# Princic-1837592/julia-raytracer

Hardware: AMD Instinct MI355X
Metric: Mrays/s + wall-clock render time, cornellbox 1280×720×256spp (higher is better)
Workload: dtype f32; 1 GPU; cornellbox path 1280x720x256spp; scene=cornellbox, sampler=path, width=1280, height=720, spp=256, bounces=8, batch=256, traversal=near, traversal_requested=auto, bvh=middle, parallelism=1 tile groups x 1 sample ranges + RCCL reduce

## Files before the change

### julia-raytracer_amd/csrc/jt_device.h

```cpp
#pragma once

#include <hip/hip_runtime.h>
#include <stdint.h>

#include "jt_records.h"

namespace jtd {

static constexpr float pif = 3.14159265358979323846f;
static constexpr float ray_eps = 0.0001f;
static constexpr float min_roughness = 0.03f * 0.03f;

struct v2 {
    float x, y;
};
struct v3 {
    float x, y, z;
};
struct v4 {
    float x, y, z, w;
};

__device__ __forceinline__ v2 V2(float x, float y) { return v2{x, y}; }
__device__ __forceinline__ v3 V3(float x, float y, float z) { return v3{x, y, z}; }
__device__ __forceinline__ v4 V4(float x, float y, float z, float w) { return v4{x, y, z, w}; }
__device__ __forceinline__ v3 operator+(v3 a, v3 b) { return V3(a.x + b.x, a.y + b.y, a.z + b.z); }
__device__ __forceinline__ v3 operator-(v3 a, v3 b) { return V3(a.x - b.x, a.y - b.y, a.z - b.z); }
__device__ __forceinline__ v3 operator*(v3 a, v3 b) { return V3(a.x * b.x, a.y * b.y, a.z * b.z); }
__device__ __forceinline__ v3 operator*(v3 a, float s) { return V3(a.x * s, a.y * s, a.z * s); }
__device__ __forceinline__ v3 operator/(v3 a, float s) { return V3(a.x / s, a.y / s, a.z / s); }
__device__ __forceinline__ v3 operator-(v3 a) { return V3(-a.x, -a.y, -a.z); }
__device__ __forceinline__ v4 operator+(v4 a, v4 b) { return V4(a.x + b.x, a.y + b.y, a.z + b.z, a.w + b.w); }
__device__ __forceinline__ v4 operator*(v4 a, float s) { return V4(a.x * s, a.y * s, a.z * s, a.w * s); }
__device__ __forceinline__ bool is_zero(v3 a) { return a.x == 0 && a.y == 0 && a.z == 0; }
__device__ __forceinline__ bool all_finite(v3 a) {
    return __builtin_isfinite(a.x) && __builtin_isfinite(a.y) && __builtin_isfinite(a.z);
}
__device__ __forceinline__ v3 xyz(float4 a) { return V3(a.x, a.y, a.z); }
__device__ __forceinline__ v3 xyz(v4 a) { return V3(a.x, a.y, a.z); }

__device__ __forceinline__ float dot(v3 a, v3 b) { return (a.x * b.x + a.y * b.y) + a.z * b.z; }
__device__ __forceinline__ v3 cross(v3 a, v3 b) {
    return V3(a.y * b.z - a.z * b.y, a.z * b.x - a.x * b.z, a.x * b.y - a.y * b.x);
}
#ifndef JT_SQRT_FORM
#define JT_SQRT_FORM 1
#endif
constexpr unsigned JL_SQRT_LO = 0x10000000u;
constexpr unsigned JL_SQRT_HI = 0x7f800000u;
template <int FORM>
__device__ __forceinline__ float sqrt_fast(float x) {
    if constexpr (FORM == 1) {
        const float y = __builtin_amdgcn_rsqf(x);
        const float s = x * y, h = 0.5f * y;
        return __builtin_fmaf(__builtin_fmaf(-s, s, x), h, s);
    } else if constexpr (FORM == 2) {
        const float s = __builtin_amdgcn_sqrtf(x), h = 0.5f * __builtin_amdgcn_rsqf(x);
        return __builtin_fmaf(__builtin_fmaf(-s, s, x), h, s);
    } else if constexpr (FORM == 3) {
        const float s = __builtin_amdgcn_sqrtf(x);
        const float dn = __uint_as_float(__float_as_uint(s) - 1u), up = __uint_as_float(__float_as_uint(s) + 1u);
        const float rd = __builtin_fmaf(-dn, s, x), ru = __builtin_fmaf(-up, s, x);
        const float t = rd <= 0.0f ? dn : s;
        return ru > 0.0f ? up : t;
    } else {
        const float y = __builtin_amdgcn_rsqf(x);
        float g = x * y, h = 0.5f * y;
        const float e = __builtin_fmaf(-h, g, 0.5f);
        h = __builtin_fmaf(h, e, h);
        g = __builtin_fmaf(g, e, g);
        return __builtin_fmaf(__builtin_fmaf(-g, g, x), h, g);
    }
}
__device__ __forceinline__ float jl_sqrt(float x) {
#if JT_SQRT_FORM
    if (__builtin_expect(__float_as_uint(x) - JL_SQRT_LO < JL_SQRT_HI - JL_SQRT_LO, 1)) return sqrt_fast<JT_SQRT_FORM>(x);
#endif
    return __builtin_sqrtf(x);
}
__device__ __forceinline__ v3 normalize(v3 a) {
    float l = jl_sqrt(dot(a, a));
    return l != 0 ? a / l : a;
}
// ... 400 lines not shown
```

### julia-raytracer_amd/csrc/jt_host.cpp

```cpp
#include <algorithm>
#include <cstdlib>
#include <cstring>
#include <mutex>
#include <string>
#include <thread>
#include <vector>

#include "jt_internal.h"

namespace jt {

static thread_local std::string g_last_error;

void set_error(const std::string& msg) { g_last_error = msg; }
int fail(int status, const std::string& msg) {
    set_error(msg);
    return status;
}

static std::mutex g_opt_mu;
static std::map<std::string, std::string> g_opts;
static const char* const kOptionNames[] = {
    "env_alias",  "features",    "lds_scene",   "lds_stack",  "light_inline", "streams",
    "wait_lanes", "light_lanes", "multi_split", "tile_share",  "test_lds_ring",
};
std::map<std::string, std::string> options_snapshot() {
    std::lock_guard<std::mutex> g(g_opt_mu);
    return g_opts;
}

frame3 inverse_frame(const frame3& f, bool non_rigid) {
    f3 c1 = f.x, c2 = f.y, c3 = f.z;
    f3 m1, m2, m3;
    if (non_rigid) {
        f3 k1 = cross(c2, c3), k2 = cross(c3, c1), k3 = cross(c1, c2);
        f3 a1 = mk3(k1.x, k2.x, k3.x), a2 = mk3(k1.y, k2.y, k3.y), a3 = mk3(k1.z, k2.z, k3.z);
        float det = dot(c1, cross(c2, c3));
        float s = 1.0f / det;
        m1 = a1 * s;
        m2 = a2 * s;
        m3 = a3 * s;
    } else {
        m1 = mk3(c1.x, c2.x, c3.x);
        m2 = mk3(c1.y, c2.y, c3.y);
        m3 = mk3(c1.z, c2.z, c3.z);
    }
    f3 t = (m1 * f.o.x + m2 * f.o.y) + m3 * f.o.z;
    return frame3{m1, m2, m3, -t};
}

struct bbox {
    f3 mn, mx;
};
static inline bbox empty_bbox() {
    const float inf = INFINITY;
    return bbox{mk3(inf, inf, inf), mk3(-inf, -inf, -inf)};
}
static inline bbox merge(const bbox& b, f3 p) {
    return bbox{mk3(jl_min(b.mn.x, p.x), jl_min(b.mn.y, p.y), jl_min(b.mn.z, p.z)),
                mk3(jl_max(b.mx.x, p.x), jl_max(b.mx.y, p.y), jl_max(b.mx.z, p.z))};
}
static inline bbox merge(const bbox& a, const bbox& b) {
    return bbox{mk3(jl_min(a.mn.x, b.mn.x), jl_min(a.mn.y, b.mn.y), jl_min(a.mn.z, b.mn.z)),
                mk3(jl_max(a.mx.x, b.mx.x), jl_max(a.mx.y, b.mx.y), jl_max(a.mx.z, b.mx.z))};
}
static inline f3 center(const bbox& b) { return (b.mn + b.mx) / 2.0f; }
static inline float bbox_area(const bbox& b) {
    f3 s = b.mx - b.mn;
    return ((0.000000000001f + 2 * s.x * s.y) + 2 * s.x * s.z) + 2 * s.y * s.z;
}

struct Builder {
    const std::vector<bbox>& boxes;
    bool hq;
    std::vector<int32_t> prims;
    std::vector<f3> centers;
    std::vector<jt_bvh_node> nodes;
// ... 410 lines not shown
```

### julia-raytracer_amd/csrc/jt_integrator.h

```cpp
#pragma once

#include <hip/hip_runtime.h>

#include "jt_bsdf.h"
#include "jt_device.h"
#include "jt_launch.h"
#include "jt_scene_eval.h"
#include "jt_traverse.h"

#ifndef JT_FUSED_BSDF
#define JT_FUSED_BSDF 1
#endif

namespace jtk {
using namespace jtd;

template <int F>
__device__ __forceinline__ v3 sample_lights(const DScene& S, v3 position, float rl, float rel, v2 ruv) {
    const int light_id = sample_uniform(S.nlights, rl);
    const DLight l = S.lights[light_id - 1];
    const float* cdf = S.cdf + l.cdf_offset;
    if (l.instance >= 0) {
        const int element = l.nguide ? sample_discrete_guided(cdf, l.ncdf, rel, S.guide_t + l.guide_offset,
                                                              S.guide_a + l.guide_offset, l.nguide, l.guide_scale)
// ... 110 lines not shown
    Volume vol;
};

__device__ __forceinline__ bool next_bounce(const DParams& P, Path& st) {
    if (st.bounce() >= P.bounces) return true;
    st.ctl += 1u;
    st.phase = PH_SCENE;
    return false;
}
__device__ __forceinline__ bool next_bounce_retry(const DParams& P, Path& st) {
    if (st.bounce() - 1 >= P.bounces) return true;
    st.phase = PH_SCENE;
    return false;
}
template <int F>
__device__ __forceinline__ bool after_weight(const DParams& P, Path& st) {
    if (is_zero(st.weight<F>()) || !all_finite(st.weight<F>())) return true;
    if (st.bounce() > 3) {
        float rr_prob = jl_min(0.99f, max3(st.weight<F>()));
        if (rand1f(st.rng) >= rr_prob) return true;
        st.set_weight<F>(st.weight<F>() * jl_rcp_weight(rr_prob));
    }
    return next_bounce(P, st);
}
template <int F>
__device__ __forceinline__ bool light_advance(const DScene& S, const DParams& P, Path& st) {
    for (;;) {
        st.li += 1;
        if (st.li >= S.nlights) {
            st.o = st.lq<F>();
            const float pdf = st.pdf * S.light_pick_pdf;
            st.set_weight<F>(st.weight<F>() / (0.5f * st.pb<F>() + 0.5f * pdf));
            return after_weight<F>(P, st);
        }
        const DLight l = S.lights[st.li];
        if (!(F & FT_NOIL) && l.instance >= 0) {
            st.lpdf = 0.0f;
            st.ctl &= (1u << CTL_LC) - 1u;
            st.o = st.lq<F>();
            st.phase = PH_LIGHT;
            return false;
        }
        if ((F & FT_ENV) && l.environment >= 0) st.pdf += env_light_pdf(S, l, st.d);
    }
}
template <int F>
__device__ __forceinline__ bool begin_light_pdf(const DScene& S, const DParams& P, Path& st) {
    st.pdf = 0.0f;
    st.li = -1;
    st.set_lq<F>(st.o);
    return light_advance<F>(S, P, st);
}
template <int F>
__device__ __forceinline__ bool light_hit_add(const DScene& S, Path& st, const Hit& h) {
    const int4 lh = row16<F>(S.light_hit + st.li);
    const DInstShade& is = S.inst_shade[lh.x];
    const fr3 f = frame_from(is.f0, is.f1, is.f2);
    const float4* r = S.light_elems + 5 * (lh.y + h.elem);
    const float4 r0 = r[0], r1 = r[1], r2 = r[2], r3 = r[3];
    const v3 p1 = V3(r0.x, r0.y, r0.z), p2 = V3(r0.w, r1.x, r1.y), p3 = V3(r1.z, r1.w, r2.x);
    const v2 uv = V2(h.u, h.v);
    v3 lposition;
    if (!(F & FT_QUAD) || __float_as_int(r3.z) == KIND_TRI) {
        lposition = transform_point(f, interp_tri(p1, p2, p3, uv));
    } else {
        const float4 r4 = r[4];
        lposition = transform_point(f, interp_quad(p1, p2, p3, V3(r4.x, r4.y, r4.z), uv));
    }
    const v3 en = V3(r2.y, r2.z, r2.w);
    v3 lnormal = __float_as_int(r3.y) ? en : transform_normal(f, en);
    const float area = r3.x;
    v3 dd = lposition - st.lq<F>();
    st.lpdf += dot(dd, dd) / (__builtin_fabsf(dot(lnormal, st.d)) * area);
    st.o = lposition + st.d * 0.001f;
    st.ctl += 1u << CTL_LC;
    return st.lcount() < 100;
}
template <int F>
__device__ __forceinline__ bool light_chain_end(const DScene& S, const DParams& P, Path& st) {
    st.pdf += st.lpdf;
    return light_advance<F>(S, P, st);
}
template <int F>
__device__ __forceinline__ bool light_hit(const DScene& S, const DParams& P, Path& st, const Hit& h) {
    if (h.hit && light_hit_add<F>(S, st, h)) return false;
    return light_chain_end<F>(S, P, st);
}

#ifndef JT_LIGHT_LEAF_STEP
#define JT_LIGHT_LEAF_STEP 1
#endif
#ifndef JT_CHAIN_TAIL
#define JT_CHAIN_TAIL 2
#endif
__host__ __device__ constexpr bool ft_mesh_kernel(int F) { return mesh_family(F); }
template <bool WIDE, int F>
__host__ __device__ constexpr bool chain_tail() {
    return JT_CHAIN_TAIL && !WIDE && !(F & FT_NOIL) && F != FT_NONE && !ft_mesh_kernel(F);
}
template <bool WIDE, bool OVF, bool NCACHE, int F>
__host__ __device__ constexpr bool chain_leaf_step() {
    return JT_LIGHT_LEAF_STEP && !WIDE && !OVF && !NCACHE && !ft_mesh_kernel(F);
}
template <bool WIDE, bool OVF, bool NCACHE, int F>
__host__ __device__ constexpr bool chain_dinv_once() {
    return JT_CHAIN_TAIL >= 2 && chain_tail<WIDE, F>() && chain_leaf_step<WIDE, OVF, NCACHE, F>();
}
// ... 133 lines not shown
        } else {
            float rnl = rand1f(st.rng);
            incoming = sample_delta<F>(sh.mat, sh.normal, outgoing, rnl);
            v3 f = eval_delta<F>(sh.mat, sh.normal, outgoing, incoming);
            float pd = sample_delta_pdf<F>(sh.mat, sh.normal, outgoing, incoming);
            st.set_weight<F>((st.weight<F>() * f) / pd);
        }
        const int mtype = sh.mat.type;
        if ((F & FT_VOL) && (mtype == M_REFRACTIVE || mtype == M_VOLUMETRIC || mtype == M_SUBSURFACE) &&
            dot(sh.normal, outgoing) * dot(sh.normal, incoming) < 0) {
            if (!st.flag(F_VOLUME)) {
                st.set_flag(F_VOLUME);
                st.vol.density = sh.mat.density;
                st.vol.scattering = sh.mat.scattering;
                st.vol.scanisotropy = sh.mat.scanisotropy;
            } else {
                st.clear_flag(F_VOLUME);
            }
        }
        st.o = sh.position;
        st.d = incoming;
        return delta ? after_weight<F>(P, st) : begin_light_pdf<F>(S, P, st);
    }
    v3 outgoing = -st.d;
    v3 position = st.o + st.d * isec.t;
    v3 incoming;
    if (rand1f(st.rng) < 0.5f) {
        (void)rand1f(st.rng);
        v2 rn = rand2f(st.rng);
        incoming = sample_scattering(st.vol, outgoing, rn);
    } else {
        float rl = rand1f(st.rng), rel = rand1f(st.rng);
        v2 ruv = rand2f(st.rng);
        incoming = sample_lights<F>(S, position, rl, rel, ruv);
    }
    if (is_zero(incoming)) return true;
    st.set_weight<F>(st.weight<F>() * eval_scattering(st.vol, outgoing, incoming));
    st.set_pb<F>(sample_scattering_pdf(st.vol, outgoing, incoming));
    st.o = position;
    st.d = incoming;
    return begin_light_pdf<F>(S, P, st);
}

template <int F, class AovT>
__device__ __forceinline__ bool naive_hit(const DScene& S, const DParams& P, Path& st, Hit isec, const AovT& aov,
                                          unsigned& shades) {
    if (!isec.hit) {
        if (st.bounce() > 0 || !P.envhidden)
            st.set_radiance<F>(st.radiance<F>() + st.weight<F>() * eval_environment<F>(S, st.d));
        return true;
    }
    v3 outgoing = -st.d;
    Shading sh;
    eval_shading<F>(S, isec.inst, isec.elem, V2(isec.u, isec.v), outgoing, sh);
    shades++;
    if ((F & FT_OPAC) && sh.mat.opacity < 1 && rand1f(st.rng) >= sh.mat.opacity) {
        if (st.opbounce() > 128) return true;
        st.ctl += 1u << CTL_OPB;
        st.o = sh.position + st.d * 0.01f;
        return next_bounce_retry(P, st);
    }
    if (st.bounce() == 0) {
        st.set_flag(F_HIT);
        aov_update<F>(aov, sh.mat.color, sh.normal);
    }
    st.set_radiance<F>(st.radiance<F>() + st.weight<F>() * (dot(sh.normal, outgoing) >= 0 ? sh.mat.emission : V3(0, 0, 0)));
    v3 incoming, f;
    float p;
    if (sh.mat.roughness != 0) {
        float rnl = rand1f(st.rng);
        v2 rn = rand2f(st.rng);
        incoming = sample_bsdfcos<F>(sh.mat, sh.normal, outgoing, rnl, rn);
        if (is_zero(incoming)) return true;
#if JT_FUSED_BSDF
        eval_bsdfcos_pdf<F>(sh.mat, sh.normal, outgoing, incoming, f, p);
#else
        f = eval_bsdfcos<F>(sh.mat, sh.normal, outgoing, incoming);
        p = sample_bsdfcos_pdf<F>(sh.mat, sh.normal, outgoing, incoming);
#endif
    } else {
        float rnl = rand1f(st.rng);
        incoming = sample_delta<F>(sh.mat, sh.normal, outgoing, rnl);
        if (is_zero(incoming)) return true;
        f = eval_delta<F>(sh.mat, sh.normal, outgoing, incoming);
        p = sample_delta_pdf<F>(sh.mat, sh.normal, outgoing, incoming);
    }
    st.set_weight<F>((st.weight<F>() * f) / p);
    st.o = sh.position;
    st.d = incoming;
    return after_weight<F>(P, st);
}

__device__ __forceinline__ void eval_camera(const DCamera& cam, v2 image_uv, v2 lens_uv, v3& ro, v3& rd) {
    const fr3 frame = frame_from(cam.frame);
    const v2 film = V2(cam.film_x, cam.film_y);
    if (!cam.orthographic) {
        v3 q = V3(film.x * (0.5f - image_uv.x), film.y * (image_uv.y - 0.5f), cam.lens);
        v3 dc = -normalize(q);
        v3 e = V3(lens_uv.x * cam.aperture / 2, lens_uv.y * cam.aperture / 2, 0);
        v3 p = (dc * cam.focus) / __builtin_fabsf(dc.z);
        v3 d = normalize(p - e);
        ro = transform_point(frame, e);
        rd = transform_direction(frame, d);
    } else {
        float scale = 1 / cam.lens;
        v3 q = V3(film.x * (0.5f - image_uv.x) * scale, film.y * (image_uv.y - 0.5f) * scale, cam.lens);
        v3 e = V3(-q.x, -q.y, 0) + V3(lens_uv.x * cam.aperture / 2, lens_uv.y * cam.aperture / 2, 0);
// ... 35 lines not shown
```

### julia-raytracer_amd/csrc/jt_layout.cpp

```cpp
#include "jt_layout.h"

#include <algorithm>
#include <cmath>
#include <cstdlib>
#include <cstring>
#include <functional>
#include <string>
#include <vector>

using namespace jtd;

namespace jt {
namespace {

inline float4 f4(float x, float y, float z, float w) { return make_float4(x, y, z, w); }
template <class I>
inline float as_f(I v) {
    static_assert(sizeof(I) == 4, "32-bit integers only");
    float f;
    std::memcpy(&f, &v, 4);
    return f;
}

void build_alias_table(const float* cdf, int n, std::vector<float2>& out) {
// ... 588 lines not shown
        const DInstShade& is = hs.inst_shade[inst];
        const DShape& d = hs.shapes[is.shape];
        const jt_shape& sh = scene->shapes[is.shape];
        const int nel = d.kind == KIND_TRI ? sh.ntriangles : sh.nquads;
        const float area = lights->lights[k].ncdf > 0 ? lights->lights[k].cdf[lights->lights[k].ncdf - 1] : 0.0f;
        hs.light_hit[k] = make_int4(inst, (int)(lelems.size() / 5), 0, 0);
        for (int e = 0; e < nel; e++) {
            const int g = d.idx_base + e;
            const int4 v = hs.elems[g];
            const float4 p1 = hs.pos[v.x], p2 = hs.pos[v.y], p3 = hs.pos[v.z];
            const float4 p4 = d.kind == KIND_TRI ? f4(0, 0, 0, 0) : hs.pos[v.w];
            const float4 n = is.rot_identity ? hs.enrm_id[g] : hs.enrm[g];
            lelems.push_back(f4(p1.x, p1.y, p1.z, p2.x));
            lelems.push_back(f4(p2.y, p2.z, p3.x, p3.y));
            lelems.push_back(f4(p3.z, n.x, n.y, n.z));
            lelems.push_back(f4(area, as_f(is.rot_identity ? 1 : 0), as_f(d.kind), 0));
            lelems.push_back(f4(p4.x, p4.y, p4.z, 0));
        }
    }
    if (lelems.empty()) lelems.assign(5, f4(0, 0, 0, 0));
}

int light_inline(const jt_scene* scene, const jt_scene_bvh* bvh, const jt_lights* lights, const Options& opts) {
    bool inl = true;
    for (int k = 0; k < lights->nlights; k++) {
        const int i0 = lights->lights[k].instance;
        if (i0 < 0) continue;
        const jt_bvh_tree& t = bvh->blas[scene->instances[i0].shape];
        inl = inl && t.nnodes > 0 && !t.nodes[0].internal;
    }
    const char* li = opt(opts, "light_inline");
    if (li && std::atoi(li) == 0) inl = false;
    return inl ? 1 : 0;
}

void pack_blob(HostScene& hs) {
    std::vector<uint4>& blob = hs.blob;
    auto add = [&](const void* data, size_t bytes) {
        const int off = (int)blob.size();
        const size_t n16 = (bytes + 15) / 16;
        blob.resize(blob.size() + std::max<size_t>(1, n16));
        if (bytes) std::memcpy(blob.data() + off, data, bytes);
        return off;
    };
#define JT_PACK(T, name) hs.S.o_##name = add(hs.name.data(), hs.name.size() * sizeof(T));
#define JT_SKIP(T, name)
    JT_SCENE_ARRAYS(JT_PACK, JT_SKIP)
#undef JT_PACK
#undef JT_SKIP
}

}

int make_wide(HostScene& hs, const jt_scene* scene, const jt_scene_bvh* bvh) {
    hs.wroot.assign(scene->nshapes, 0);
    const int r = build_wide(bvh->tlas, [&](int k) -> unsigned {
        const jt_bvh_node& n = bvh->tlas.nodes[k];
        return W_LEAF | W_INST | (unsigned)(n.num - 1) << 28 | (unsigned)hs.tleaf_start[k];
    }, hs.wnodes);
    if (r < 0) return JT_ERR_UNSUPPORTED;
    hs.S.tlas_wnodes = (int)hs.wnodes.size();
    for (int s = 0; s < scene->nshapes; s++) {
        const jt_bvh_tree& t = bvh->blas[s];
        hs.wroot[s] = build_wide(t, [&](int k) -> unsigned {
            const int st0 = hs.leaf_rec[s][k];
            if (st0 < 0 || st0 > (int)IDX_MASK) return jt::fail(JT_ERR_UNSUPPORTED, "wide traversal: too many primitive records"), (unsigned)W_EMPTY;
            return W_LEAF | (unsigned)(t.nodes[k].num - 1) << 28 | (unsigned)st0;
        }, hs.wnodes);
        if (hs.wroot[s] < 0) return JT_ERR_UNSUPPORTED;
    }
    for (size_t k0 = 0; k0 < hs.inst_blas.size(); k0++) hs.inst_blas[hs.inst_new[k0]].x = hs.wroot[scene->instances[k0].shape];
    hs.wide = true;
    return JT_OK;
}

int layout_scene(const jt_scene* scene, const jt_scene_bvh* bvh, const jt_lights* lights, const jt_params* params,
                 const Options& opts, HostScene& hs) {
    if (!scene || !bvh || !lights || !params) return jt::fail(JT_ERR_INVALID, "NULL argument");
    hs = HostScene{};
    int st;
    if ((st = validate(scene, bvh, lights, params)) || (st = renumber_instances(scene, bvh, hs)) ||
        (st = stack_bound(scene, bvh, params, hs)))
        return st;
    int32_t W = 0, H = 0;
    if ((st = jt_image_size(scene, params, &W, &H)) != JT_OK) return st;
    hs.width = W;
    hs.height = H;
    hs.feat = scene_features(scene, opts);

    flatten_tlas(bvh->tlas, hs);
    hs.shapes.resize(scene->nshapes);
    hs.leaf_rec.resize(scene->nshapes);
    for (int s = 0; s < scene->nshapes; s++) {
        flatten_shape(scene->shapes[s], hs, hs.shapes[s]);
        flatten_blas(scene->shapes[s], bvh->blas[s], hs.shapes[s], hs, hs.leaf_rec[s]);
    }
    if (params->traversal < JT_TRAVERSAL_REFERENCE || params->traversal > JT_TRAVERSAL_AUTO)
        return jt::fail(JT_ERR_INVALID, "traversal must be 0 (reference), 1 (near), 2 (wide) or 3 (auto)");
    hs.wroot.assign(scene->nshapes, 0);
    if (params->traversal == JT_TRAVERSAL_WIDE && (st = make_wide(hs, scene, bvh)) != JT_OK) return st;
    flatten_instances(scene, bvh, hs);
    if ((st = flatten_materials(scene, hs)) != JT_OK) return st;
    const char* ea = opt(opts, "env_alias");
    hs.env_alias = ea && std::atoi(ea) != 0;
    flatten_lights(scene, lights, hs);
    build_luts(hs.srgb_lut, hs.byte_lut);

    for (int q = 0; q < 4; q++) hs.prims.push_back(f4(0, 0, 0, 0));
    if (hs.wide) hs.nodes.clear();
    if (hs.nodes.size() > IDX_MASK || (size_t)scene->ninstances > IDX_MASK)
        return jt::fail(JT_ERR_UNSUPPORTED, "scene exceeds 2^24 BVH nodes or instances");
    DScene& S = hs.S;
    S.order_flip = params->traversal == JT_TRAVERSAL_REFERENCE ? 0 : 7;
    S.nenvs = scene->nenvironments;
    S.nlights = lights->nlights;
    S.light_pick_pdf = lights->nlights > 0 ? (float)(1.0 / (double)lights->nlights) : 0.0f;
    S.light_inline = light_inline(scene, bvh, lights, opts);
    pack_blob(hs);
    return JT_OK;
}

}
```

### julia-raytracer_amd/csrc/jt_layout.h

```cpp
#pragma once

#include <map>
#include <string>
#include <vector>

#include "jt_internal.h"
#include "jt_records.h"

#define JT_SCENE_ARRAYS(BLOB, HBM)                                                                      \
    BLOB(jtd::DNode, nodes) BLOB(jtd::DWide, wnodes) BLOB(float4, prims) BLOB(jtd::DInstTrav, inst_trav) \
    BLOB(int4, inst_blas) BLOB(jtd::DInstShade, inst_shade) BLOB(jtd::DShape, shapes) BLOB(float4, pos)  \
    BLOB(float4, nrm) BLOB(float2, tc) BLOB(float4, col) BLOB(int4, elems) BLOB(float4, enrm)            \
    BLOB(float4, enrm_id) BLOB(jtd::DMaterial, materials) HBM(jtd::DTexture, textures) HBM(uchar4, texb) \
    HBM(float4, texf) HBM(jtd::DEnv, envs) BLOB(jtd::DLight, lights) BLOB(float, cdf)                    \
    BLOB(int4, light_hit) BLOB(float4, light_elems) HBM(float, guide_t) HBM(int, guide_a)                \
    HBM(float2, alias) HBM(float, srgb_lut) HBM(float, byte_lut)

namespace jt {

using Options = std::map<std::string, std::string>;
inline const char* opt(const Options& opts, const char* k) {
    const auto it = opts.find(k);
    return it == opts.end() ? nullptr : it->second.c_str();
}

using jtk::IDX_MASK;

struct HostScene {
#define JT_ARRAY_VECTOR(T, name) std::vector<T> name;
    JT_SCENE_ARRAYS(JT_ARRAY_VECTOR, JT_ARRAY_VECTOR)
#undef JT_ARRAY_VECTOR
    std::vector<uint4> blob;
    jtd::DScene S{};
    int need = 0;
    int feat = jtd::FT_ALL;
    int width = 0, height = 0;
    bool wide = false;
    bool env_alias = false;
    bool inst_light = false;
    std::vector<int> inst_new, tleaf_start, wroot;
    std::vector<std::vector<int>> leaf_rec;
};

int layout_scene(const jt_scene* scene, const jt_scene_bvh* bvh, const jt_lights* lights, const jt_params* params,
                 const Options& opts, HostScene& hs);
int make_wide(HostScene& hs, const jt_scene* scene, const jt_scene_bvh* bvh);

}
```

### julia-raytracer_amd/csrc/jt_records.h

```cpp
#pragma once

#include <hip/hip_vector_types.h>
#include <stdint.h>

#include "jt_plan.h"
#include "jt_select.h"

#define JT_DEFER_SAMPLES 64
#ifndef JT_EXACT_MATH
#define JT_EXACT_MATH 1
#endif

namespace jtd {

struct alignas(16) DNode {
    float4 a, b;
};
struct alignas(16) DWide {
    float4 r0;
    uint4 r1, r2;
    uint4 r3;
};
enum : unsigned { W_EMPTY = 0xffffffffu, W_LEAF = 0x80000000u, W_INST = 0x40000000u, W_START = 0x0fffffffu };
struct alignas(16) DInstTrav {
    float4 i0, i1, i2;
    int shape, blas_root, kind, prim_base;
};
struct alignas(16) DInstShade {
    float4 f0, f1, f2;
    int material, shape, mat_type;
    int rot_identity;
};
enum { KIND_TRI = 0, KIND_QUAD = 1 };
struct alignas(16) DShape {
    int kind, blas_root, prim_base, idx_base;
    int pos_base, nrm_base, tc_base, col_base;
};
struct alignas(16) DMaterial {
    int type, emission_tex, color_tex, roughness_tex;
    int scattering_tex, normal_tex, pad0, pad1;
    float emission[3], roughness;
    float color[3], metallic;
    float scattering[3], ior;
    float scanisotropy, trdepth, opacity, pad2;
};
struct alignas(16) DTexture {
    int width, height, linear, is_float;
    long long offset;
    long long pad;
};
struct alignas(16) DEnv {
    float frame[12];
    float inv[12];
    float emission[3];
    int tex;
};
struct alignas(16) DLight {
    int instance, environment, cdf_offset, ncdf;
    int guide_offset, nguide;
    float guide_scale;
    int alias_offset;
};

struct DScene {
    const DNode* nodes;
    const DWide* wnodes;
    int tlas_wnodes;
    const float4* prims;
    const DInstTrav* inst_trav;
    const int4* inst_blas;
    const DInstShade* inst_shade;
    const DShape* shapes;
    const float4* pos;
    const float4* nrm;
    const float2* tc;
    const float4* col;
    const int4* elems;
    const float4* enrm;
    const float4* enrm_id;
    const DMaterial* materials;
    const DTexture* textures;
    const uchar4* texb;
    const float4* texf;
    const DEnv* envs;
    const DLight* lights;
    const int4* light_hit;
    const float4* light_elems;
    const float* cdf;
    const float* guide_t;
    const int* guide_a;
    const float2* alias;
    const float* srgb_lut;
    const float* byte_lut;
    int tlas_nnodes, nenvs, nlights;
    int order_flip;
    float light_pick_pdf;
    int light_inline;
    const uint4* blob;
    int blob_n16;
    int* ovf;
    int ovf_stride;
    int ring;
    int stack_need;
    int o_wnodes;
    int o_nodes, o_prims, o_inst_trav, o_inst_blas, o_inst_shade, o_shapes;
    int o_pos, o_nrm, o_tc, o_col, o_elems, o_materials, o_lights, o_cdf, o_enrm, o_enrm_id;
    int o_light_hit, o_light_elems;
};

struct DCamera {
    float frame[12];
    int orthographic;
    float lens, film, aspect, focus, aperture;
    float film_x, film_y;
    int pinhole;
};

struct DParams {
    DCamera cam;
    int width, height;
// ... 14 lines not shown
```

### julia-raytracer_amd/csrc/jt_scene_eval.h

```cpp
#pragma once

#include <hip/hip_runtime.h>

#include "jt_bsdf.h"
#include "jt_device.h"

namespace jtk {
using namespace jtd;

template <int F>
__device__ __forceinline__ int4 row16(const void* p) {
    int4 v = *reinterpret_cast<const int4*>(p);
    if (!ft_none(F)) __asm__("" : "+v"(v.x), "+v"(v.y), "+v"(v.z), "+v"(v.w));
    return v;
}
template <int F>
__device__ __forceinline__ int4 inst_ids(const DScene& S, int inst) {
    return row16<F>(reinterpret_cast<const char*>(S.inst_shade + inst) + 48);
}
__device__ __forceinline__ fr3 inst_frame(const DScene& S, int inst) {
    const DInstShade& r = S.inst_shade[inst];
    return frame_from(r.f0, r.f1, r.f2);
}

template <int F>
__device__ __forceinline__ v3 eval_position(const DScene& S, int inst, int elem, v2 uv) {
    const DInstShade& is = S.inst_shade[inst];
    const int4 sh = row16<F>(S.shapes + inst_ids<F>(S, inst).y);
    const int4 e = S.elems[sh.w + elem];
    const fr3 f = frame_from(is.f0, is.f1, is.f2);
    v3 p1 = xyz(S.pos[e.x]), p2 = xyz(S.pos[e.y]), p3 = xyz(S.pos[e.z]);
    if (!(F & FT_QUAD) || sh.x == KIND_TRI) return transform_point(f, interp_tri(p1, p2, p3, uv));
    return transform_point(f, interp_quad(p1, p2, p3, xyz(S.pos[e.w]), uv));
}
__device__ __forceinline__ v3 element_normal(const DScene& S, int rot_identity, const fr3& f, int g) {
    const v3 n = xyz((rot_identity ? S.enrm_id : S.enrm)[g]);
    return rot_identity ? n : transform_normal(f, n);
}
template <int F>
__device__ __forceinline__ v3 eval_element_normal(const DScene& S, int inst, int elem) {
    const DInstShade& is = S.inst_shade[inst];
    const int4 ids = inst_ids<F>(S, inst);
    const int4 sh = row16<F>(S.shapes + ids.y);
    return element_normal(S, ids.w, frame_from(is.f0, is.f1, is.f2), sh.w + elem);
}
__device__ __forceinline__ v3 eval_normal(const DScene& S, const DShape& sh, const int4& e, const fr3& f, v2 uv) {
    if (sh.nrm_base < 0) {
        v3 p1 = xyz(S.pos[e.x]), p2 = xyz(S.pos[e.y]), p3 = xyz(S.pos[e.z]);
        if (sh.kind == KIND_TRI) return transform_normal(f, triangle_normal(p1, p2, p3));
        return transform_normal(f, quad_normal(p1, p2, p3, xyz(S.pos[e.w])));
    }
    const int b = sh.nrm_base - sh.pos_base;
    v3 n1 = xyz(S.nrm[e.x + b]), n2 = xyz(S.nrm[e.y + b]), n3 = xyz(S.nrm[e.z + b]);
    if (sh.kind == KIND_TRI) return transform_normal(f, normalize(interp_tri(n1, n2, n3, uv)));
    return transform_normal(f, normalize(interp_quad(n1, n2, n3, xyz(S.nrm[e.w + b]), uv)));
}
__device__ __forceinline__ v2 eval_texcoord(const DScene& S, const DShape& sh, const int4& e, v2 uv) {
    if (sh.tc_base < 0) return uv;
    const int b = sh.tc_base - sh.pos_base;
    float2 t1 = S.tc[e.x + b], t2 = S.tc[e.y + b], t3 = S.tc[e.z + b];
    if (sh.kind == KIND_TRI) return interp_tri(V2(t1.x, t1.y), V2(t2.x, t2.y), V2(t3.x, t3.y), uv);
    float2 t4 = S.tc[e.w + b];
    return interp_quad(V2(t1.x, t1.y), V2(t2.x, t2.y), V2(t3.x, t3.y), V2(t4.x, t4.y), uv);
}
__device__ __forceinline__ v4 eval_color(const DScene& S, const DShape& sh, const int4& e, v2 uv) {
    if (sh.col_base < 0) return V4(1, 1, 1, 1);
    const int b = sh.col_base - sh.pos_base;
    float4 c1 = S.col[e.x + b], c2 = S.col[e.y + b], c3 = S.col[e.z + b];
    v4 a = V4(c1.x, c1.y, c1.z, c1.w), bb = V4(c2.x, c2.y, c2.z, c2.w), c = V4(c3.x, c3.y, c3.z, c3.w);
    if (sh.kind == KIND_TRI) return interp_tri(a, bb, c, uv);
    float4 c4 = S.col[e.w + b];
    return interp_quad(a, bb, c, V4(c4.x, c4.y, c4.z, c4.w), uv);
}
__device__ __forceinline__ v4 lookup_texture(const DScene& S, const DTexture& t, int i, int j, bool as_linear) {
    long long k = t.offset + (long long)j * t.width + i;
    if (t.is_float) {
        float4 c = S.texf[k];
        return V4(c.x, c.y, c.z, c.w);
    }
    uchar4 b = S.texb[k];
    const float* lut = (as_linear && !t.linear) ? S.srgb_lut : S.byte_lut;
    return V4(lut[b.x], lut[b.y], lut[b.z], S.byte_lut[b.w]);
// ... 37 lines not shown
        const TexelPair r1 = *reinterpret_cast<const TexelPair*>(S.texb + t.offset + (long long)jj * t.width + i);
        uchar4 c0 = r0.b, c1 = r1.b;
        if (ii == 0) {
            c0 = S.texb[t.offset + (long long)j * t.width];
            c1 = S.texb[t.offset + (long long)jj * t.width];
        }
        const float* lut = tex_lut + ((as_linear && !t.linear) ? 0 : 256);
        ta = decode_texel(r0.a, lut);
        tb = decode_texel(r1.a, lut);
        tc = decode_texel(c0, lut);
        td = decode_texel(c1, lut);
    }
    v4 a = (ta * (1 - u)) * (1 - v);
    v4 b = (tb * (1 - u)) * v;
    v4 c = (tc * u) * (1 - v);
    v4 d = (td * u) * v;
    return ((a + b) + c) + d;
}
__device__ __forceinline__ v3 eval_normalmap(const DScene& S, const DShape& sh, const int4& e, const fr3& f,
                                          const DMaterial& m, v2 uv) {
    v3 normal = eval_normal(S, sh, e, f, uv);
    v2 texcoord = eval_texcoord(S, sh, e, uv);
    v4 t4 = eval_texture(S, m.normal_tex, texcoord, false);
    v3 nm = V3(t4.x * 2 - 1, t4.y * 2 - 1, t4.z * 2 - 1);
    v3 tu = V3(0, 0, 0), tv = V3(0, 0, 0);
    if (sh.tc_base >= 0) {
        const int b = sh.tc_base - sh.pos_base;
        float2 a1 = S.tc[e.x + b], a2 = S.tc[e.y + b];
        if (sh.kind == KIND_TRI) {
            float2 a3 = S.tc[e.z + b];
            triangle_tangents_fromuv(xyz(S.pos[e.x]), xyz(S.pos[e.y]), xyz(S.pos[e.z]), V2(a1.x, a1.y),
                                     V2(a2.x, a2.y), V2(a3.x, a3.y), tu, tv);
        } else {
            float2 a4 = S.tc[e.w + b];
            triangle_tangents_fromuv(xyz(S.pos[e.x]), xyz(S.pos[e.y]), xyz(S.pos[e.w]), V2(a1.x, a1.y),
                                     V2(a2.x, a2.y), V2(a4.x, a4.y), tu, tv);
        }
        tu = transform_direction(f, tu);
        tv = transform_direction(f, tv);
    }
    v3 f1 = normalize(tu - normal * dot(tu, normal));
    v3 f2 = normalize(cross(normal, tu));
    bool flip_v = dot(f2, tv) < 0;
    nm = V3(nm.x, nm.y * (flip_v ? 1.0f : -1.0f), nm.z);
    fr3 fr{f1, f2, normal, V3(0, 0, 0)};
    return transform_normal(fr, nm);
}

struct Shading {
    v3 position, normal;
    MatPoint mat;
};

template <int F>
__device__ __forceinline__ void eval_shading(const DScene& S, int inst, int elem, v2 uv, v3 outgoing, Shading& out) {
    const DInstShade is = S.inst_shade[inst];
    const DShape sh = S.shapes[is.shape];
    const int4 e = S.elems[sh.idx_base + elem];
    const fr3 f = frame_from(is.f0, is.f1, is.f2);
    const DMaterial& m = S.materials[is.material];
    v3 p1 = xyz(S.pos[e.x]), p2 = xyz(S.pos[e.y]), p3 = xyz(S.pos[e.z]);
    const bool tri = !(F & FT_QUAD) || sh.kind == KIND_TRI;
    v3 p4 = !tri ? xyz(S.pos[e.w]) : p3;
    out.position = tri ? transform_point(f, interp_tri(p1, p2, p3, uv))
                       : transform_point(f, interp_quad(p1, p2, p3, p4, uv));
    const int mtype = (F & FT_MAT) ? m.type : (int)M_MATTE;
    v3 normal;
    if ((F & FT_TEX) && m.normal_tex >= 0) {
        normal = eval_normalmap(S, sh, e, f, m, uv);
    } else if (!(F & FT_ATTR) || sh.nrm_base < 0) {
        normal = element_normal(S, is.rot_identity, f, sh.idx_base + elem);
    } else {
        normal = eval_normal(S, sh, e, f, uv);
    }
    if (mtype != M_REFRACTIVE) normal = dot(normal, outgoing) >= 0 ? normal : -normal;
    out.normal = normal;
    MatPoint& p = out.mat;
    const v4 one = V4(1, 1, 1, 1);
    v2 texcoord = (F & FT_ATTR) ? eval_texcoord(S, sh, e, uv) : uv;
    v4 emission_tex = (F & FT_TEX) ? eval_texture(S, m.emission_tex, texcoord, true) : one;
    v4 color_shp = (F & FT_ATTR) ? eval_color(S, sh, e, uv) : one;
    v4 color_tex = (F & FT_TEX) ? eval_texture(S, m.color_tex, texcoord, true) : one;
    v4 roughness_tex = (F & FT_TEX) ? eval_texture(S, m.roughness_tex, texcoord, false) : one;
    v4 scattering_tex = (F & FT_TEX) ? eval_texture(S, m.scattering_tex, texcoord, true) : one;
    p.type = mtype;
    p.emission = V3(m.emission[0], m.emission[1], m.emission[2]) * xyz(emission_tex);
    p.color = (V3(m.color[0], m.color[1], m.color[2]) * xyz(color_tex)) * xyz(color_shp);
    p.opacity = m.opacity * color_tex.w * color_shp.w;
    p.metallic = m.metallic * roughness_tex.z;
    float roughness = m.roughness * roughness_tex.y;
    roughness = roughness * roughness;
    p.ior = m.ior;
    p.scattering = V3(m.scattering[0], m.scattering[1], m.scattering[2]) * xyz(scattering_tex);
    p.scanisotropy = m.scanisotropy;
    p.trdepth = m.trdepth;
    if ((F & FT_VOL) && (mtype == M_REFRACTIVE || mtype == M_VOLUMETRIC || mtype == M_SUBSURFACE)) {
        p.density = V3(-jl_log(jl_clamp(p.color.x, 0.0001f, 1.0f)) / p.trdepth,
                       -jl_log(jl_clamp(p.color.y, 0.0001f, 1.0f)) / p.trdepth,
                       -jl_log(jl_clamp(p.color.z, 0.0001f, 1.0f)) / p.trdepth);
    } else {
        p.density = V3(0, 0, 0);
    }
    if (mtype == M_MATTE || mtype == M_GLTFPBR || mtype == M_GLOSSY) roughness = jl_clamp(roughness, min_roughness, 1.0f);
    else if (mtype == M_VOLUMETRIC) roughness = 0.0f;
    else if (roughness < min_roughness) roughness = 0.0f;
    p.roughness = roughness;
}

template <int F>
__device__ __forceinline__ v3 eval_environment(const DScene& S, v3 direction) {
    v3 emission = V3(0, 0, 0);
    if (!(F & FT_ENV)) return emission;
    for (int k = 0; k < S.nenvs; k++) {
        const DEnv& env = S.envs[k];
        v3 wl = transform_direction(frame_from(env.inv), direction);
        v2 tc = V2(jl_atan2(wl.z, wl.x) / (2.0f * pif), jl_acos(jl_clamp(wl.y, -1.0f, 1.0f)) / pif);
        if (tc.x < 0.0f) tc.x = tc.x + 1.0f;
        v4 t = eval_texture(S, env.tex, tc, false);
        emission = emission + V3(env.emission[0], env.emission[1], env.emission[2]) * xyz(t);
    }
    return emission;
}

}
// ... 1 lines not shown
```

### julia-raytracer_amd/csrc/jt_trace.hip

```cpp
#include <hip/hip_runtime.h>

#include <algorithm>
#include <array>
#include <cassert>
#include <cmath>
#include <cstdio>
#include <cstdlib>
#include <cstring>
#include <string>
#include <utility>
#include <vector>

#include "jt_accum.h"
#include "jt_context.h"
#include "jt_layout.h"

using namespace jtd;
using namespace jtk;
using namespace jtc;

namespace {
using LaunchFn = hipError_t (*)(const DScene&, const DParams&, int, int, const DAccum&, hipStream_t, int);
struct LaunchRow {
    LaunchFn fn[2][2][2];
// ... 594 lines not shown
    if (c->multi) return multi_get_counters(c, out);
    (void)hipSetDevice(c->device);
    unsigned long long v[8] = {0};
    hipError_t e = hipMemcpy(v, c->A.counters, 7 * 8, hipMemcpyDeviceToHost);
    if (e != hipSuccess) return hip_fail(e, "hipMemcpy counters");
    out->paths = v[0];
    out->rays = v[1];
    out->light_queries = v[2];
    out->nodes = v[3];
    out->instances = v[4];
    out->prims = v[5];
    out->shades = v[6];
    out->launches = c->launches;
    out->kernel_ms = c->kernel_ms;
    return JT_OK;
}

int jt_get_device_buffers(jt_ctx* c, jt_device_buffers* out) {
    if (!c || !out) return jt::fail(JT_ERR_INVALID, "NULL argument");
    if (const int st = flush(c)) return st;
    if (c->multi) return multi_get_device_buffers(c, out);
    if (const int st = zero_if_stale(c)) return st;
    if (const int st = finish_aovs(c)) return st;
    c->exported = true;
    out->image = c->A.image;
    out->albedo = c->A.albedo;
    out->normal = c->A.normal;
    out->hits = c->A.hits;
    out->width = c->width;
    out->height = c->height;
    out->stream = c->stream;
    return JT_OK;
}

extern "C" int jt_debug_stamps(jt_ctx* c, unsigned long long* out8) {
    if (!c || !out8) return jt::fail(JT_ERR_INVALID, "NULL argument");
    hipError_t e = hipMemcpy(out8, c->A.counters + 8, 24 * 8, hipMemcpyDeviceToHost);
    return e == hipSuccess ? JT_OK : hip_fail(e, "hipMemcpy stamps");
}

int jt_describe(const jt_ctx* c, char* buf, int32_t n) {
    if (!c || !buf || n <= 0) return jt::fail(JT_ERR_INVALID, "NULL argument");
    if (c->multi) return multi_describe(c, buf, n);
    const KernelChoice& k = c->choice;
    char filt[96] = "";
    if (c->P.tile_stride != 1 || k.ring_shortened())
        std::snprintf(filt, sizeof filt, " tile_filter=%d/%d ring_used=%d", c->P.tile_offset, c->P.tile_stride, c->S.ring);
    char adaptive[48] = "";
    if (c->adapted) std::snprintf(adaptive, sizeof adaptive, " adaptive=%d/%d", c->adapt_active, launch_tiles(c->P));
    char tmp[704];
    std::snprintf(tmp, sizeof tmp,
                  "kernel=%s<%d,%d,%s,%d,%d,%s> mode=%s scene_lds_bytes=%zu stack_bound=%d lds_ring=%d hbm_overflow=%d "
                  "wait_lanes=%d light_lanes=%d streams=%d tiles=%d block=%d env_alias=%d light_inline=%d "
                  "traversal=%s%s%s",
                  k.lds_scene_bytes ? "trace_kernel_lds" : "trace_kernel", c->sampler == JT_SAMPLER_NAIVE ? 2 : 1,
                  k.ring, k.ovf ? "true" : "false", c->count, k.kmask, k.wide ? "true" : "false",
                  k.lds_scene_bytes ? "lds" : "hbm", k.lds_scene_bytes,
                  k.stack, k.ring, k.ovf ? 1 : 0, c->P.wait_lanes, c->P.light_lanes, 1 << c->lk, c->tiles, BLOCK,
                  c->env_alias ? 1 : 0, c->S.light_inline,
                  k.traversal == JT_TRAVERSAL_REFERENCE ? "reference" : k.traversal == JT_TRAVERSAL_NEAR ? "near" : "wide",
                  filt, adaptive);
    std::snprintf(buf, (size_t)n, "%s", tmp);
    return JT_OK;
}

int jt_set_counters(jt_ctx* c, int32_t level) {
    if (!c) return jt::fail(JT_ERR_INVALID, "ctx is NULL");
    if (level != 0 && level != 1) return jt::fail(JT_ERR_INVALID, "counter level must be 0 or 1");
    if (const int st = flush(c)) return st;
    if (c->multi) return multi_set_counters(c, level);
    c->count = level;
    return JT_OK;
}

int jt_synchronize(jt_ctx* c) {
    if (!c) return jt::fail(JT_ERR_INVALID, "ctx is NULL");
    if (const int st = flush(c)) return st;
    if (c->multi) return multi_synchronize(c);
    if (const int st = finish_aovs(c)) return st;
    (void)hipSetDevice(c->device);
    hipError_t e = hipStreamSynchronize(c->stream);
    return e == hipSuccess ? JT_OK : hip_fail(e, "hipStreamSynchronize");
}

}
```

Before: 13920 Mrays/s.

## Skip instance transforms when every instance frame is identity

At scene upload, the host checks whether every instance frame is exactly the identity and all positions are finite. If so, it sets a point_identity flag. The path-tracer shading, position evaluation and light-hit code then skip the frame transform and read precomputed element normals directly. An optional shared-denominator vec3 division path is also added behind JT_DIV3, which is off by default. The flag adds a runtime branch and extra code paths. Bitwise-identical results are kept by adding 0.0f instead of calling transform_point.

```diff
diff --git a/julia-raytracer_amd/csrc/jt_device.h b/julia-raytracer_amd/csrc/jt_device.h
--- a/julia-raytracer_amd/csrc/jt_device.h
+++ b/julia-raytracer_amd/csrc/jt_device.h
@@ -28,7 +28,37 @@
 __device__ __forceinline__ v3 operator-(v3 a, v3 b) { return V3(a.x - b.x, a.y - b.y, a.z - b.z); }
 __device__ __forceinline__ v3 operator*(v3 a, v3 b) { return V3(a.x * b.x, a.y * b.y, a.z * b.z); }
 __device__ __forceinline__ v3 operator*(v3 a, float s) { return V3(a.x * s, a.y * s, a.z * s); }
-__device__ __forceinline__ v3 operator/(v3 a, float s) { return V3(a.x / s, a.y / s, a.z / s); }
+#ifndef JT_DIV3
+#define JT_DIV3 0
+#endif
+__device__ __forceinline__ bool div3_dens_equal(v3 a, float b, float& d) {
+    bool unused;
+    d = __builtin_amdgcn_div_scalef(a.x, b, false, &unused);
+    const float dy = __builtin_amdgcn_div_scalef(a.y, b, false, &unused);
+    const float dz = __builtin_amdgcn_div_scalef(a.z, b, false, &unused);
+    const unsigned differ = (__float_as_uint(d) ^ __float_as_uint(dy)) | (__float_as_uint(d) ^ __float_as_uint(dz));
+    return __builtin_amdgcn_ballot_w64(differ != 0u) == 0;
+}
+__device__ __forceinline__ float div3_tail(float n, float b, float d, float y) {
+    bool vcc;
+    const float sn = __builtin_amdgcn_div_scalef(n, b, true, &vcc);
+    float q = sn * y;
+    float r = __builtin_fmaf(-d, q, sn);
+    q = __builtin_fmaf(r, y, q);
+    r = __builtin_fmaf(-d, q, sn);
+    return __builtin_amdgcn_div_fixupf(__builtin_amdgcn_div_fmasf(r, y, q, vcc), b, n);
+}
+__device__ __forceinline__ v3 operator/(v3 a, float s) {
+#if JT_DIV3
+    float d;
+    if (__builtin_expect(div3_dens_equal(a, s, d), 1)) {
+        float y = __builtin_amdgcn_rcpf(d);
+        y = __builtin_fmaf(__builtin_fmaf(-d, y, 1.0f), y, y);
+        return V3(div3_tail(a.x, s, d, y), div3_tail(a.y, s, d, y), div3_tail(a.z, s, d, y));
+    }
+#endif
+    return V3(a.x / s, a.y / s, a.z / s);
+}
 __device__ __forceinline__ v3 operator-(v3 a) { return V3(-a.x, -a.y, -a.z); }
 __device__ __forceinline__ v4 operator+(v4 a, v4 b) { return V4(a.x + b.x, a.y + b.y, a.z + b.z, a.w + b.w); }
 __device__ __forceinline__ v4 operator*(v4 a, float s) { return V4(a.x * s, a.y * s, a.z * s, a.w * s); }
diff --git a/julia-raytracer_amd/csrc/jt_host.cpp b/julia-raytracer_amd/csrc/jt_host.cpp
--- a/julia-raytracer_amd/csrc/jt_host.cpp
+++ b/julia-raytracer_amd/csrc/jt_host.cpp
@@ -22,7 +22,7 @@
 static std::map<std::string, std::string> g_opts;
 static const char* const kOptionNames[] = {
     "env_alias",  "features",    "lds_scene",   "lds_stack",  "light_inline", "streams",
-    "wait_lanes", "light_lanes", "multi_split", "tile_share",  "test_lds_ring",
+    "wait_lanes", "light_lanes", "multi_split", "tile_share",  "test_lds_ring", "point_identity",
 };
 std::map<std::string, std::string> options_snapshot() {
     std::lock_guard<std::mutex> g(g_opt_mu);
diff --git a/julia-raytracer_amd/csrc/jt_integrator.h b/julia-raytracer_amd/csrc/jt_integrator.h
--- a/julia-raytracer_amd/csrc/jt_integrator.h
+++ b/julia-raytracer_amd/csrc/jt_integrator.h
@@ -186,7 +186,32 @@
     return light_advance<F>(S, P, st);
 }
 template <int F>
+__device__ __forceinline__ bool light_hit_add_identity(const DScene& S, Path& st, const Hit& h) {
+    const int4 lh = row16<F>(S.light_hit + st.li);
+    const float4* r = S.light_elems + 5 * (lh.y + h.elem);
+    const float4 r0 = r[0], r1 = r[1], r2 = r[2], r3 = r[3];
+    const v3 p1 = V3(r0.x, r0.y, r0.z), p2 = V3(r0.w, r1.x, r1.y), p3 = V3(r1.z, r1.w, r2.x);
+    const v2 uv = V2(h.u, h.v);
+    v3 lposition;
+    if (!(F & FT_QUAD) || __float_as_int(r3.z) == KIND_TRI) {
+        lposition = identity_point(interp_tri(p1, p2, p3, uv));
+    } else {
+        const float4 r4 = r[4];
+        lposition = identity_point(interp_quad(p1, p2, p3, V3(r4.x, r4.y, r4.z), uv));
+    }
+    const v3 lnormal = V3(r2.y, r2.z, r2.w);
+    const float area = r3.x;
+    v3 dd = lposition - st.lq<F>();
+    st.lpdf += dot(dd, dd) / (__builtin_fabsf(dot(lnormal, st.d)) * area);
+    st.o = lposition + st.d * 0.001f;
+    st.ctl += 1u << CTL_LC;
+    return st.lcount() < 100;
+}
+template <int F>
 __device__ __forceinline__ bool light_hit_add(const DScene& S, Path& st, const Hit& h) {
+    if constexpr (point_identity_kernel<F>()) {
+        if (S.point_identity) return light_hit_add_identity<F>(S, st, h);
+    }
     const int4 lh = row16<F>(S.light_hit + st.li);
     const DInstShade& is = S.inst_shade[lh.x];
     const fr3 f = frame_from(is.f0, is.f1, is.f2);
@@ -426,7 +451,7 @@
     }
     v3 outgoing = -st.d;
     Shading sh;
-    eval_shading<F>(S, isec.inst, isec.elem, V2(isec.u, isec.v), outgoing, sh);
+    eval_shading<F, false>(S, isec.inst, isec.elem, V2(isec.u, isec.v), outgoing, sh);
     shades++;
     if ((F & FT_OPAC) && sh.mat.opacity < 1 && rand1f(st.rng) >= sh.mat.opacity) {
         if (st.opbounce() > 128) return true;
diff --git a/julia-raytracer_amd/csrc/jt_layout.cpp b/julia-raytracer_amd/csrc/jt_layout.cpp
--- a/julia-raytracer_amd/csrc/jt_layout.cpp
+++ b/julia-raytracer_amd/csrc/jt_layout.cpp
@@ -664,6 +664,21 @@
 
 }
 
+bool frame_point_identity(const float* fv) {
+    const float id[12] = {1, 0, 0, 0, 1, 0, 0, 0, 1, 0, 0, 0};
+    return std::memcmp(fv, id, sizeof id) == 0;
+}
+bool scene_point_identity(const jt_scene* scene) {
+    for (int k = 0; k < scene->ninstances; k++)
+        if (!frame_point_identity(scene->instances[k].frame)) return false;
+    for (int s = 0; s < scene->nshapes; s++) {
+        const jt_shape& sh = scene->shapes[s];
+        for (size_t q = 0; q < (size_t)sh.npositions * 3; q++)
+            if (!(std::fabs(sh.positions[q]) < 0x1p125f)) return false;
+    }
+    return true;
+}
+
 int make_wide(HostScene& hs, const jt_scene* scene, const jt_scene_bvh* bvh) {
     hs.wroot.assign(scene->nshapes, 0);
     const int r = build_wide(bvh->tlas, [&](int k) -> unsigned {
@@ -728,6 +743,8 @@
     S.nlights = lights->nlights;
     S.light_pick_pdf = lights->nlights > 0 ? (float)(1.0 / (double)lights->nlights) : 0.0f;
     S.light_inline = light_inline(scene, bvh, lights, opts);
+    const char* pi = opt(opts, "point_identity");
+    S.point_identity = scene_point_identity(scene) && !(pi && std::atoi(pi) == 0) ? 1 : 0;
     pack_blob(hs);
     return JT_OK;
 }
diff --git a/julia-raytracer_amd/csrc/jt_layout.h b/julia-raytracer_amd/csrc/jt_layout.h
--- a/julia-raytracer_amd/csrc/jt_layout.h
+++ b/julia-raytracer_amd/csrc/jt_layout.h
@@ -46,4 +46,7 @@
                  const Options& opts, HostScene& hs);
 int make_wide(HostScene& hs, const jt_scene* scene, const jt_scene_bvh* bvh);
 
+bool frame_point_identity(const float* fv);
+bool scene_point_identity(const jt_scene* scene);
+
 }
diff --git a/julia-raytracer_amd/csrc/jt_records.h b/julia-raytracer_amd/csrc/jt_records.h
--- a/julia-raytracer_amd/csrc/jt_records.h
+++ b/julia-raytracer_amd/csrc/jt_records.h
@@ -66,6 +66,7 @@
     const DNode* nodes;
     const DWide* wnodes;
     int tlas_wnodes;
+    int point_identity;
     const float4* prims;
     const DInstTrav* inst_trav;
     const int4* inst_blas;
diff --git a/julia-raytracer_amd/csrc/jt_scene_eval.h b/julia-raytracer_amd/csrc/jt_scene_eval.h
--- a/julia-raytracer_amd/csrc/jt_scene_eval.h
+++ b/julia-raytracer_amd/csrc/jt_scene_eval.h
@@ -23,11 +23,27 @@
     return frame_from(r.f0, r.f1, r.f2);
 }
 
+#ifndef JT_POINT_IDENTITY
+#define JT_POINT_IDENTITY 1
+#endif
+template <int F, bool PID = true>
+__host__ __device__ constexpr bool point_identity_kernel() {
+    return PID && JT_POINT_IDENTITY && !(F & FT_XFORM);
+}
+__device__ __forceinline__ v3 identity_point(v3 p) { return V3(p.x + 0.0f, p.y + 0.0f, p.z + 0.0f); }
+
 template <int F>
 __device__ __forceinline__ v3 eval_position(const DScene& S, int inst, int elem, v2 uv) {
     const DInstShade& is = S.inst_shade[inst];
     const int4 sh = row16<F>(S.shapes + inst_ids<F>(S, inst).y);
     const int4 e = S.elems[sh.w + elem];
+    if constexpr (point_identity_kernel<F>()) {
+        if (S.point_identity) {
+            v3 p1 = xyz(S.pos[e.x]), p2 = xyz(S.pos[e.y]), p3 = xyz(S.pos[e.z]);
+            if (!(F & FT_QUAD) || sh.x == KIND_TRI) return identity_point(interp_tri(p1, p2, p3, uv));
+            return identity_point(interp_quad(p1, p2, p3, xyz(S.pos[e.w]), uv));
+        }
+    }
     const fr3 f = frame_from(is.f0, is.f1, is.f2);
     v3 p1 = xyz(S.pos[e.x]), p2 = xyz(S.pos[e.y]), p3 = xyz(S.pos[e.z]);
     if (!(F & FT_QUAD) || sh.x == KIND_TRI) return transform_point(f, interp_tri(p1, p2, p3, uv));
@@ -171,7 +187,7 @@
     MatPoint mat;
 };
 
-template <int F>
+template <int F, bool PID = true>
 __device__ __forceinline__ void eval_shading(const DScene& S, int inst, int elem, v2 uv, v3 outgoing, Shading& out) {
     const DInstShade is = S.inst_shade[inst];
     const DShape sh = S.shapes[is.shape];
@@ -181,14 +197,27 @@
     v3 p1 = xyz(S.pos[e.x]), p2 = xyz(S.pos[e.y]), p3 = xyz(S.pos[e.z]);
     const bool tri = !(F & FT_QUAD) || sh.kind == KIND_TRI;
     v3 p4 = !tri ? xyz(S.pos[e.w]) : p3;
-    out.position = tri ? transform_point(f, interp_tri(p1, p2, p3, uv))
-                       : transform_point(f, interp_quad(p1, p2, p3, p4, uv));
+    bool pid = false;
+    if constexpr (point_identity_kernel<F, PID>()) {
+        pid = S.point_identity != 0;
+        const v3 pobj = tri ? interp_tri(p1, p2, p3, uv) : interp_quad(p1, p2, p3, p4, uv);
+        if (pid) out.position = identity_point(pobj);
+        else out.position = transform_point(f, pobj);
+    } else {
+        out.position = tri ? transform_point(f, interp_tri(p1, p2, p3, uv))
+                           : transform_point(f, interp_quad(p1, p2, p3, p4, uv));
+    }
     const int mtype = (F & FT_MAT) ? m.type : (int)M_MATTE;
     v3 normal;
     if ((F & FT_TEX) && m.normal_tex >= 0) {
         normal = eval_normalmap(S, sh, e, f, m, uv);
     } else if (!(F & FT_ATTR) || sh.nrm_base < 0) {
-        normal = element_normal(S, is.rot_identity, f, sh.idx_base + elem);
+        if constexpr (point_identity_kernel<F, PID>()) {
+            if (pid) normal = xyz(S.enrm_id[sh.idx_base + elem]);
+            else normal = element_normal(S, is.rot_identity, f, sh.idx_base + elem);
+        } else {
+            normal = element_normal(S, is.rot_identity, f, sh.idx_base + elem);
+        }
     } else {
         normal = eval_normal(S, sh, e, f, uv);
     }
diff --git a/julia-raytracer_amd/csrc/jt_trace.hip b/julia-raytracer_amd/csrc/jt_trace.hip
--- a/julia-raytracer_amd/csrc/jt_trace.hip
+++ b/julia-raytracer_amd/csrc/jt_trace.hip
@@ -670,12 +670,12 @@
     std::snprintf(tmp, sizeof tmp,
                   "kernel=%s<%d,%d,%s,%d,%d,%s> mode=%s scene_lds_bytes=%zu stack_bound=%d lds_ring=%d hbm_overflow=%d "
                   "wait_lanes=%d light_lanes=%d streams=%d tiles=%d block=%d env_alias=%d light_inline=%d "
-                  "traversal=%s%s%s",
+                  "point_identity=%d traversal=%s%s%s",
                   k.lds_scene_bytes ? "trace_kernel_lds" : "trace_kernel", c->sampler == JT_SAMPLER_NAIVE ? 2 : 1,
                   k.ring, k.ovf ? "true" : "false", c->count, k.kmask, k.wide ? "true" : "false",
                   k.lds_scene_bytes ? "lds" : "hbm", k.lds_scene_bytes,
                   k.stack, k.ring, k.ovf ? 1 : 0, c->P.wait_lanes, c->P.light_lanes, 1 << c->lk, c->tiles, BLOCK,
-                  c->env_alias ? 1 : 0, c->S.light_inline,
+                  c->env_alias ? 1 : 0, c->S.light_inline, c->S.point_identity,
                   k.traversal == JT_TRAVERSAL_REFERENCE ? "reference" : k.traversal == JT_TRAVERSAL_NEAR ? "near" : "wide",
                   filt, adaptive);
     std::snprintf(buf, (size_t)n, "%s", tmp);
```

Result: no change. 14000 Mrays/s, median of 6 (+0.5%).
